# koesterlab/microphaser

Measured on AMD Instinct MI355X. Metric: peptide-windows/s (somatic, 9-mer), higher is better.
Workload: dtype u64

## Files before the change

### microphaser_amd/csrc/capi.cpp

```cpp
#include "../../include/microphaser_hip.h"

#include <cstdio>
#include <cstdlib>
#include <cstring>
#include <chrono>
#include <unistd.h>
#include <cerrno>
#include <fstream>
#include <iostream>
#include <memory>
#include <sstream>

#include "batch.hpp"
#include "consume.hpp"
#include "device.hpp"
#include "filter.hpp"
#include "pep.hpp"
#include "synth.hpp"

using namespace mp;

#include "capi_types.hpp"


// ... 193 lines not shown
                    batch->w_wins_known = true;
                }
                const uint64_t w_steps = batch->w_steps;
                const uint64_t seq_steps = b.steps.size() - w_steps, seq_wins = b.wins.size() - batch->w_wins;
                const double wfrac = b.wins.empty() ? 0.0 : double(batch->w_wins) / double(b.wins.size());
                const uint64_t groups_w = uint64_t(double(t.n_groups) * wfrac), groups_seq = t.n_groups - groups_w;
                const uint64_t read_bytes = 20 + 16ull * b.mask_words;
                st->k2seq_ms = t.k2seq_ms; st->k2a_ms = t.k2a_ms; st->k2w_ms = t.k2w_ms; st->k2win_ms = t.k2win_ms;
                st->n_steps_seq = seq_steps; st->n_steps_w = w_steps; st->n_adm = b.n_adm;
                const uint64_t rowrec = b.lane_on ? sizeof(RowRecA) + 8 : 0;
                if (!batch->adm_known) {
                    for (const ExonW& e : b.exons_w) { if (e.consumers & EW_WAVE) batch->adm_wave += e.n_reads; if (e.consumers & EW_LANE) batch->adm_lane += e.n_reads; }
                    batch->adm_known = true;
                }
                st->bytes_k2a = b.n_adm * read_bytes + batch->adm_wave * sizeof(AdmEntry) + batch->adm_lane * rowrec + b.exons_w.size() * sizeof(ExonW);
                uint64_t wave_steps = 0;
                for (const PodVec<WChunk>* list : {&b.wchunks, &b.wchunks_m, &b.wchunks_d}) for (const WChunk& c : *list) wave_steps += c.n_steps;
                const double wave_share = w_steps ? double(wave_steps) / double(w_steps) : 0.0;
                const uint64_t lane_wins = b.winw.size(), wave_wins = batch->w_wins - std::min<uint64_t>(batch->w_wins, lane_wins);
                const uint64_t groups_l = batch->w_wins ? uint64_t(double(groups_w) * double(lane_wins) / double(batch->w_wins)) : 0;
                st->k2l_ms = t.k2l_ms; st->n_windows_lane = lane_wins; st->n_windows_wave = wave_wins;
                const uint64_t listed_l = t.n_k3 > (t.n_groups - groups_l) ? t.n_k3 - (t.n_groups - groups_l) : 0;
                st->bytes_k2l = lane_wins * (sizeof(WinW) + 4 + sizeof(WinDyn)) + batch->adm_lane * rowrec + groups_l * sizeof(Group) + listed_l * 16;
                st->bytes_k2w = wave_steps * (sizeof(Step) + 7) + uint64_t(double(b.n_adm) * wave_share) * (read_bytes + sizeof(AdmEntry)) +
                                wave_wins * sizeof(WinDyn) + (groups_w - groups_l) * (sizeof(Group) + 16);
                st->bytes_k2seq = seq_steps * sizeof(Step) + (b.steps.empty() ? 0 : uint64_t(double(b.r_pos.size()) * double(seq_steps) / double(b.steps.size()))) * read_bytes +
                                  seq_wins * sizeof(WinDyn) + groups_seq * (sizeof(Group) + 16);
                st->bytes_k2 = st->bytes_k2a + st->bytes_k2l + st->bytes_k2w + st->bytes_k2seq;
            }
            st->n_groups_k3 = t.n_k3;
// ... 334 lines not shown
```

### microphaser_amd/csrc/device.cpp

```cpp
#include "device.hpp"
#include <chrono>
#include <cstdio>
#include <algorithm>

#include <algorithm>
#include <cstdlib>
#include <cstring>
#include <thread>

namespace mp {

[[noreturn]] void throw_hip(hipError_t e, const char* file, int line) {
    throw Error(std::string("HIP error: ") + hipGetErrorString(e) + " at " + file + ":" + std::to_string(line));
}
#define HIP_OK(x) do { hipError_t e_ = (x); if (e_ != hipSuccess) throw_hip(e_, __FILE__, __LINE__); } while (0)

DeviceContext::DeviceContext(int device) : device_(device) {
    int n = 0;
    hipError_t e = hipGetDeviceCount(&n);
    if (e != hipSuccess || n == 0) throw Error("no HIP device available: the phasing hot path needs an MI355X (gfx950); there is no CPU fallback");
    if (device < 0 || device >= n) throw Error("invalid HIP device index " + std::to_string(device));
    HIP_OK(hipSetDevice(device));
    HIP_OK(hipStreamCreateWithFlags(&stream_, hipStreamNonBlocking));
    for (auto& ev : ev_) HIP_OK(hipEventCreate(&ev));
// ... 271 lines not shown
    d_.tx_first_stop = static_cast<uint32_t*>(dalloc(size_t(d_.n_tx) * 4)); allocs_.push_back(d_.tx_first_stop);
    max_rows_bound_ = b.max_rows_bound;
    last_slots_ = last_recs_ = last_want_ = last_k3a_ = last_k3b_ = last_k3c_ = last_k3d_ = 0;
    rpl_ = 1;
    while (rpl_ < 16 && uint32_t(64 * rpl_) < max_rows_bound_) rpl_ *= 2;
    const uint64_t waves = b.wchunks.size() + b.segs.size() + b.wchunks_m.size() * (1 + b.rows_per_lane_w) + b.wchunks_d.size() * 16;
    uint64_t g_need = uint64_t(d_.n_wins) * 6 + waves * 256 + 4096;
    uint64_t r_need = g_need / 3 + waves * 128 + 4096;
    if (b.normal) { g_need += waves * 1024; r_need = g_need; }
    glog_ = 12; rlog_ = 12;
    while ((uint64_t(NPART) << glog_) < g_need + g_need / 4) glog_++;
    while ((uint64_t(NPART) << rlog_) < r_need + r_need / 4) rlog_++;
    if (std::getenv("MP_TEST_SMALL_CAPS")) glog_ = rlog_ = 8;
    d_.win_blobs = nullptr;
    if (!b.normal && d_.n_wins) { d_.win_blobs = static_cast<WinBlob*>(dalloc(size_t(d_.n_wins) * sizeof(WinBlob))); allocs_.push_back(d_.win_blobs); }
    d_.exons_a = nullptr; d_.adm_map = nullptr;
    if (b.n_adm) {
        d_.exons_a = static_cast<ExonA*>(dalloc(size_t(d_.n_exons_w) * sizeof(ExonA))); allocs_.push_back(d_.exons_a);
        d_.adm_map = static_cast<AdmMap*>(dalloc(size_t(b.n_adm) * sizeof(AdmMap))); allocs_.push_back(d_.adm_map);
    }
    const double ms_inputs = ms_since(t_up0);
    alloc_outputs();
    const double ms_alloc = ms_since(t_up0);
    uint64_t up_bytes = 0;
    for (const XferSeg& sgm : pending_up_) up_bytes += sgm.bytes;
    if (dbg) {
        std::vector<uint64_t> sz;
        for (const XferSeg& sgm : pending_up_) sz.push_back(sgm.bytes);
        std::sort(sz.rbegin(), sz.rend());
        std::fprintf(stderr, "[mp]   upload: %zu arrays, %.2f GB; the largest (MB):", pending_up_.size(), double(up_bytes) / 1e9);
        for (size_t k = 0; k < sz.size() && k < 14; k++) std::fprintf(stderr, " %.0f", double(sz[k]) / 1e6);
        std::fprintf(stderr, "\n[mp]   upload sizes (MB): reads fields %.0f, seq pool %.0f, cigar %.0f, ref %.0f, steps %.0f (+ side arrays %.0f), wins %.0f, win_cols %.0f, winw %.0f\n",
                     double(b.r_pos.size()) * (4 * 7 + 8 * 3) / 1e6, double(b.seq_pool.size()) / 1e6, double(b.cigar_pool.size()) * 4 / 1e6, double(b.ref_pool.size()) / 1e6,
                     double(b.steps.size()) * sizeof(Step) / 1e6, double(b.steps.size()) * 13 / 1e6 + double(b.step_aux.size()) * sizeof(b.step_aux[0]) / 1e6,
                     double(b.wins.size()) * sizeof(WinStatic) / 1e6, double(b.win_cols.size()) * sizeof(WinCol) / 1e6, double(b.winw.size()) * (sizeof(WinW) + 4) / 1e6);
    }
    xfer(pending_up_, true);
    pending_up_.clear();
    if (dbg) std::fprintf(stderr, "[mp]   upload: %u hipMalloc calls took %.1f ms in all; %u blocks came from the context's pool\n", alloc_calls_, alloc_ms_, alloc_reused_);
    if (dbg)
        std::fprintf(stderr, "[mp]   upload: release of the previous batch %.1f ms, per-read table + input allocations %.1f ms, result arenas %.1f ms, copies %.1f ms\n",
                     ms_free, ms_inputs - ms_free, ms_alloc - ms_inputs, ms_since(t_up0) - ms_alloc);
    launch_k0_read_variants(d_, stream_);
    launch_k0_pack_admission(d_, stream_);
    if (d_.win_blobs) launch_k0_pack_windows(d_, stream_);
    HIP_OK(hipStreamSynchronize(stream_));
    pool_trim(false);
}

void DeviceContext::alloc_outputs() {
    if ((uint64_t(NPART) << glog_) > 0x7FFFFFFFull || (uint64_t(NPART) << rlog_) > 0x7FFFFFFFull)
        throw Error("result buffers exceed 2^31 slots: split the batch by genes");
    free_outputs();
    group_cap_ = uint64_t(NPART) << glog_;
    rec_cap_ = uint64_t(NPART) << rlog_;
    auto oalloc = [&](size_t bytes) { void* p = dalloc(bytes); out_allocs_.push_back(p); out_bytes_ += bytes; return p; };
    d_.groups = static_cast<Group*>(oalloc(group_cap_ * sizeof(Group)));
    d_.k3_items = static_cast<uint4*>(oalloc(2 * group_cap_ * sizeof(uint4)));
    d_.gsum = static_cast<GroupSum*>(oalloc(group_cap_ * sizeof(GroupSum)));
    d_.recs = static_cast<uint8_t*>(oalloc(rec_cap_ * d_.rec_stride));
    d_.want_recs = static_cast<uint32_t*>(oalloc(rec_cap_ * 4));
    d_.group_part_log2 = glog_;
    d_.rec_part_log2 = rlog_;
    d_.group_cap = group_cap_;
    d_.rec_cap = rec_cap_;
}

void DeviceContext::run(RunTiming& t) {
    HIP_OK(hipSetDevice(device_));
    t = RunTiming();
    for (int attempt = 0; attempt < 8; attempt++) {
        t.attempts = uint32_t(attempt + 1);
        t.rows_per_lane = rpl_;
        HIP_OK(hipMemsetAsync(d_.cursors, 0, (NPART * 32 + 16) * 8, stream_));
        HIP_OK(hipMemsetAsync(d_.win_dyn, 0, size_t(d_.n_wins) * sizeof(WinDyn), side_[0]));
        HIP_OK(hipMemsetAsync(d_.tx_first_stop, 0xFF, size_t(d_.n_tx) * 4, side_[0]));
        HIP_OK(hipEventRecord(cleared_, side_[0]));
        HIP_OK(hipEventRecord(ev_[0], stream_));
        launch_k1_pileup_bits(d_, stream_);
        HIP_OK(hipEventRecord(ev_[1], stream_));
        HIP_OK(hipStreamWaitEvent(stream_, cleared_, 0));
        HIP_OK(hipEventRecord(fork_[0], stream_));
        HIP_OK(hipStreamWaitEvent(side_[2], fork_[0], 0));
        launch_k2_window_replay(d_, rpl_, side_[2]);
        HIP_OK(hipEventRecord(join_[2], side_[2]));
        HIP_OK(hipEventRecord(ev_[5], stream_));
        launch_k2_admission(d_, stream_);
        HIP_OK(hipEventRecord(ev_[6], stream_));
// ... 145 lines not shown
```

### microphaser_amd/csrc/device.hpp

```cpp
#pragma once
#include <string>
#include <vector>

#include "batch.hpp"
#include "kernels.hpp"

namespace mp {

struct HostResults {
    PodVec<WinDyn> win_dyn;
    PodVec<Group> groups;
    PodVec<GroupSum> gsum;
    PodVec<uint8_t> recs;
    uint32_t seq_cap = 48, rec_stride = 128;
    uint32_t group_part_log2 = 0, rec_part_log2 = 0;
    uint64_t group_prefix[NPART + 1] = {0}, rec_prefix[NPART + 1] = {0};
    size_t gidx(uint64_t slot) const { return size_t(group_prefix[slot >> group_part_log2] + (slot & ((1ull << group_part_log2) - 1))); }
    size_t ridx(uint64_t i) const { return size_t(rec_prefix[i >> rec_part_log2] + (i & ((1ull << rec_part_log2) - 1))); }
    const Group& grp(uint64_t slot) const { return groups[gidx(slot)]; }
    const GroupSum& gsm(uint64_t slot) const { return gsum[gidx(slot)]; }
    const HapRecHdr* rec(uint64_t i) const { return reinterpret_cast<const HapRecHdr*>(recs.data() + ridx(i) * rec_stride); }
    const uint8_t* rec_seq(uint64_t i) const { return recs.data() + ridx(i) * rec_stride + 32; }
    const uint8_t* rec_germ(uint64_t i) const { return recs.data() + ridx(i) * rec_stride + 32 + seq_cap; }
    uint64_t n_group_slots = 0, n_recs = 0;
};

struct RunTiming {
    float k1_ms = 0, k2_ms = 0, k3_ms = 0, k3b_ms = 0, total_ms = 0;
    float k2seq_ms = 0, k2a_ms = 0, k2l_ms = 0, k2w_ms = 0;
    float k2win_ms = 0;
    uint64_t n_group_slots = 0, n_recs = 0, n_groups = 0, n_k3 = 0, n_k3a = 0, n_k3c = 0, n_k3d = 0, n_rec_slots = 0;
    int rows_per_lane = 1;
    uint32_t attempts = 0;
};

class DeviceContext {
  public:
    explicit DeviceContext(int device);
    ~DeviceContext();
    DeviceContext(const DeviceContext&) = delete;
    DeviceContext& operator=(const DeviceContext&) = delete;

    void upload(const Batch& b);
    void run(RunTiming& t);
    void download(HostResults& r);
    void free_batch();
    int device() const { return device_; }
    uint64_t hbm_bytes() const { return hbm_bytes_; }
// ... 42 lines not shown
```

### microphaser_amd/csrc/kernels.hip

```cpp
#include <hip/hip_runtime.h>

#include <algorithm>
#include <cstdlib>
#include <type_traits>

#include "kernels.hpp"

namespace mp {

#ifndef MP_KPART
#define MP_KPART -1
#endif
#define MP_IN_PART(n) (MP_KPART == -1 || MP_KPART == (n))
#define HIP_CHECK_LAUNCH() \
    do { hipError_t e_ = hipGetLastError(); if (e_ != hipSuccess) { throw_hip(e_, __FILE__, __LINE__); } } while (0)

[[noreturn]] void throw_hip(hipError_t e, const char* file, int line);

#if MP_IN_PART(0)
__global__ __launch_bounds__(256) void k0_read_variants(DeviceBatch d) {
    const uint32_t i = blockIdx.x * 256u + threadIdx.x;
    if (i >= d.n_reads) return;
    uint32_t lo = 0, hi = d.n_genes;
    while (hi - lo > 1) {
// ... 62 lines not shown
    }
    return -1;
}

__device__ __forceinline__ uint8_t decode_base4(uint32_t code) {
    const uint64_t lo = 0x565352474d43413dull, hi = 0x4e42444b48595754ull;
    return uint8_t(((code & 8) ? hi : lo) >> (8 * (code & 7)));
}

constexpr uint32_t K1_LANES = 4;
static_assert(K1_LANES == 4, "the group's lanes combine their bits with quad permutes");
constexpr uint32_t K1_PAY_DW = 32;
constexpr uint32_t K1_PAY_STRIDE = 33;
struct __attribute__((packed, aligned(4))) K1Quad { uint32_t x, y, z, w; };

template <int W>
__global__ __launch_bounds__(256) void k1_pileup_bits(DeviceBatch d) {
    __shared__ uint32_t pay[(256 / K1_LANES) * K1_PAY_STRIDE];
    const uint64_t t = uint64_t(blockIdx.x) * 256u + threadIdx.x;
    const uint32_t sub = threadIdx.x & (K1_LANES - 1);
    const uint64_t i_raw = t / K1_LANES;
    const bool valid = i_raw < d.n_reads;
    const uint32_t i = valid ? uint32_t(i_raw) : d.n_reads - 1;
    const uint2 rv = d.r_var[i];
    const uint32_t vfirst = rv.x;
    const uint32_t rpos = d.r_pos[i], rend = d.r_end[i], lseq = d.r_lseq[i], ncig = d.r_ncig[i];
    const uint32_t* cig = d.cigar_pool + d.r_cigoff[i];
    const uint32_t* lowq = reinterpret_cast<const uint32_t*>(d.seq_pool + d.r_seqoff[i]);
    const uint32_t nlq = (lseq + 31) >> 5;
    const uint8_t* seq4 = reinterpret_cast<const uint8_t*>(lowq + nlq);
    const uint32_t cover_end = max(rend, rpos + lseq);
    const uint32_t maxn = min(rv.y, 64u * W);
    uint32_t* const slot = pay + (threadIdx.x / K1_LANES) * K1_PAY_STRIDE;
// ... 81 lines not shown
        ncov += __popc(acc_c);
#pragma unroll
        for (int w = 0; w < W; w++)
            if ((b0 >> 6) == uint32_t(w)) { sup[w] |= uint64_t(acc_s) << (b0 & 63u); lq[w] |= uint64_t(acc_q) << (b0 & 63u); }
        more = more && acc_c == 0xFFFFFFFFu;
    }
    };
    if (!any_long) run_batches(std::false_type{});
    else run_batches(std::true_type{});
    if (valid && sub == 0) {
        d.r_ncov[i] = ncov;
#pragma unroll
        for (int w = 0; w < W; w++) {
            d.r_sup[uint64_t(i) * W + w] = sup[w];
            d.r_lq[uint64_t(i) * W + w] = lq[w];
        }
    }
}

enum : uint32_t { ST_EMPTY = 0, ST_PENDING = 1, ST_ROW = 2, ST_MASK = 3, RF_BAD = 4, RF_SL = 8, RF_F1 = 16 };

__device__ __forceinline__ uint32_t rdlane(uint32_t v, uint32_t l) { return __builtin_amdgcn_readlane(v, l); }
__device__ __forceinline__ uint32_t lanes_below(uint64_t mask, uint32_t lane) { return __popcll(mask & ((1ull << lane) - 1ull)); }
__device__ __forceinline__ uint64_t wave_claim(unsigned long long* cur, unsigned long long want, uint64_t part_lo) {
    unsigned long long base = 0;
    if (threadIdx.x == 0) base = atomicAdd(cur, want);
    const uint32_t blo = rdlane(uint32_t(base), 0), bhi = rdlane(uint32_t(base >> 32), 0);
    return part_lo + ((uint64_t(bhi) << 32) | blo);
}

// ... 487 lines not shown
            w[8] = uint32_t(bits); w[9] = uint32_t(bits >> 32);
        }
    }
    return __ballot(lane < nb && ((w[5] >> 8) & SF_PRINT) && !k2l_takes(d.lane_on != 0, w[7] >> 16, w[7] & 0xFFFF));
}

#if MP_IN_PART(0)
__global__ __launch_bounds__(256) void k0_pack_admission(DeviceBatch d) {
    const uint64_t i = uint64_t(blockIdx.x) * 256u + threadIdx.x;
    if (i < d.n_exons_w) {
        const ExonW e = d.exons_w[i];
        ExonA a;
        a.step_off = e.step_off; a.n_steps = e.n_steps; a.unit_steps = e.unit_steps; a.sso0 = e.sso0;
        a.sso1 = e.sso1; a.first_key_lo = e.first_key_lo; a.range = e.range; a.tr0 = e.tr0;
        a.f0 = e.f0; a.sl_f_lo = e.sl_f_lo; a.sl_f_hi = e.sl_f_hi; a.flags = (e.strand ? 1u : 0u) | (e.consumers << 8);
        a.adm_off = e.adm_off; a.read0 = e.rbase + e.read_lo; a.wlen_min = e.wlen_min; a.pad1 = 0;
        d.exons_a[i] = a;
    }
    if (i < d.n_adm) {
        uint32_t lo = 0, hi = d.n_exons_w;
        while (hi - lo > 1) {
            const uint32_t mid = lo + (hi - lo) / 2;
            if (d.exons_w[mid].adm_off <= i) lo = mid; else hi = mid;
        }
        const ExonW* e = d.exons_w + lo;
        AdmMap m;
        m.exon = lo;
        m.read = e->rbase + e->read_lo + uint32_t(i - e->adm_off);
        d.adm_map[i] = m;
    }
}
void launch_k0_pack_admission(const DeviceBatch& d, hipStream_t stream) {
    if (!d.n_adm) return;
    const uint64_t n = d.n_adm > d.n_exons_w ? d.n_adm : d.n_exons_w;
    hipLaunchKernelGGL(k0_pack_admission, dim3(uint32_t((n + 255) / 256)), dim3(256), 0, stream, d);
    HIP_CHECK_LAUNCH();
}
#endif

template <int W>
__global__ __launch_bounds__(64) void k2a_admission_flat(DeviceBatch d) {
    struct In {
        bool on, rev, go;
        uint32_t entry, t;
        AdmMap xr;
        ExonA e;
        uint32_t start, end, rvl;
        uint64_t sup[W], dirty[W];
        uint32_t s_sso, s_col_hi, s_w4, s_w5, nc;
        AdmEntry out;
    };
    const uint32_t n_adm = uint32_t(d.n_adm);
    auto load_entry = [&](In& I, uint32_t tile) __attribute__((always_inline)) {
        const uint64_t entry = uint64_t(tile) * 64u + threadIdx.x;
        I.on = entry < n_adm;
        I.entry = I.on ? uint32_t(entry) : n_adm - 1u;
        I.xr = d.adm_map[I.entry];
    };
    auto load_fields = [&](In& I) __attribute__((always_inline)) {
        const uint4* ep = reinterpret_cast<const uint4*>(d.exons_a + I.xr.exon);
        const uint4 q0 = ep[0], q1 = ep[1], q2 = ep[2], q3 = ep[3];
        const uint32_t gi = I.xr.read;
        I.start = d.r_pos[gi]; I.end = d.r_end[gi]; I.rvl = d.r_varlo[gi];
#pragma unroll
        for (int w = 0; w < W; w++) { I.sup[w] = d.r_sup[uint64_t(gi) * W + w]; I.dirty[w] = d.r_lq[uint64_t(gi) * W + w]; }
        I.e.step_off = q0.x; I.e.n_steps = q0.y; I.e.unit_steps = q0.z; I.e.sso0 = q0.w;
        I.e.sso1 = q1.x; I.e.first_key_lo = q1.y; I.e.range = q1.z; I.e.tr0 = q1.w;
        I.e.f0 = q2.x; I.e.sl_f_lo = q2.y; I.e.sl_f_hi = q2.z; I.e.flags = q2.w;
        I.e.adm_off = q3.x; I.e.read0 = q3.y; I.e.wlen_min = q3.z;
    };
    auto load_step = [&](In& I, uint32_t si) __attribute__((always_inline)) {
        const uint32_t* sp = reinterpret_cast<const uint32_t*>(d.steps + si);
        I.s_sso = sp[0]; I.s_col_hi = sp[2]; I.s_w4 = sp[4]; I.s_w5 = sp[5];
        I.nc = d.step_ncols[si];
    };
    auto eval_step = [&](In& I, uint32_t si) __attribute__((always_inline)) -> bool {
        const uint32_t s_wlen = (I.s_w4 >> 16) & 0xFFu, s_nadd = I.s_w5 & 0xFFu;
        const uint32_t tlo = I.s_col_hi - I.nc, thi = I.s_col_hi - s_nadd;
        uint32_t flo = tlo, fhi = thi;
        if (I.rev) { flo = I.e.f0 - (thi - 1 - I.e.tr0); fhi = I.e.f0 - (tlo - I.e.tr0) + 1; }
        if (thi <= tlo) flo = fhi = 0;
        const bool encloses = !(I.end < I.s_sso + s_wlen) & !(I.start > I.s_sso);
        const bool clean = !mask_hits<W>(I.dirty, flo, fhi, I.rvl);
        const bool ok = encloses & clean;
        I.out.ord = ok ? si : I.out.ord;
        I.out.seen_lo = ok ? tlo : I.out.seen_lo;
        return ok;
    };
    auto first_step = [&](In& I) __attribute__((always_inline)) {
        const ExonA& e = I.e;
        I.rev = (e.flags & 1u) != 0;
#pragma unroll
        for (int w = 0; w < W; w++) I.dirty[w] |= I.sup[w] & bit_range(e.sl_f_lo, e.sl_f_hi, I.rvl + 64u * w);
        I.out.ord = 0xFFFFFFFFu; I.out.seen_lo = 0;
        I.go = false; I.t = 0;
        const uint32_t start = I.start;
        if (!I.rev) {
            if (start >= e.first_key_lo && start <= e.sso0) {
                I.go = true;
            } else if (start > e.sso0 && e.n_steps > 1 && start >= e.sso1) {
                uint32_t t = 1 + (start - e.sso1);
                if (t < e.unit_steps) { I.go = true; I.t = t; }
                else if (t < e.n_steps) {
                    uint32_t s_t = d.steps[e.step_off + t].sso;
                    while (s_t > start && t > 1) s_t = d.steps[e.step_off + --t].sso;
                    while (s_t < start && t + 1 < e.n_steps) s_t = d.steps[e.step_off + ++t].sso;
                    if (s_t == start) { I.go = true; I.t = t; }
                }
            }
        } else {
            const uint32_t top = start + e.range;
            uint32_t t = e.sso0 > top ? e.sso0 - top : 0;
            if (t >= e.unit_steps) {
                if (t >= e.n_steps) t = e.n_steps - 1;
                while (t > 0 && d.steps[e.step_off + t - 1].sso <= top) t--;
                while (t < e.n_steps && d.steps[e.step_off + t].sso > top) t++;
            }
            if (t < e.unit_steps) {
                const uint32_t need = e.sso0 + e.wlen_min > I.end ? e.sso0 + e.wlen_min - I.end : 0u;
                t = max(t, min(need, e.unit_steps));
            }
            I.go = t < e.n_steps; I.t = I.go ? t : 0;
        }
    };
    auto finish = [&](In& I) __attribute__((always_inline)) {
        const ExonA& e = I.e;
        if (I.go) {
            if (!I.rev) eval_step(I, e.step_off + I.t);
            else {
                uint32_t t = I.t;
                for (;;) {
                    if (I.s_sso < I.start) break;
                    if (eval_step(I, e.step_off + t)) break;
                    if (++t >= e.n_steps) break;
                    load_step(I, e.step_off + t);
                }
            }
        }
        if (!I.on) return;
        const uint32_t consumers = e.flags >> 8;
        if (consumers & EW_WAVE) d.adm[I.entry] = I.out;
        if constexpr (W == 1) {
            if (d.lane_on && (consumers & EW_LANE)) {
                uint32_t bad_from = 0xFFFFFFFFu;
                if (I.out.ord != 0xFFFFFFFFu) {
                    const uint64_t dm = I.dirty[0];
                    if (!I.rev) {
                        const uint32_t from = max(I.out.seen_lo, I.rvl), sh = from - I.rvl;
                        const uint64_t m = sh < 64 ? dm >> sh : 0ull;
                        if (m) bad_from = from + uint32_t(__builtin_ctzll(m));
                    } else {
                        const uint32_t f_hi = e.f0 - (I.out.seen_lo - e.tr0);
                        if (f_hi >= I.rvl) {
                            const uint32_t rel = f_hi - I.rvl;
                            const uint64_t m = rel >= 63 ? dm : (dm & ((2ull << rel) - 1ull));
                            if (m) bad_from = e.tr0 + (e.f0 - (I.rvl + 63u - uint32_t(__builtin_clzll(m))));
                        }
                    }
                }
                RowRecA a;
                a.key = I.rev ? ~I.start : I.end;
                a.ord = I.out.ord;
                a.bad_from = bad_from;
                a.rvl = I.rvl;
                d.rr_a[I.entry] = a;
                d.rr_sup[I.entry] = I.sup[0];
            }
        }
    };
    In in0;
    load_entry(in0, blockIdx.x);
    load_fields(in0);
    first_step(in0);
    load_step(in0, in0.e.step_off + in0.t);
    finish(in0);
}

template <int HB, int STAGE_>
__global__ __launch_bounds__(64) void k2l_window_lanes(DeviceBatch d, uint32_t first, uint32_t count) {
    constexpr bool HASH = HB > 8;
    constexpr uint32_t NW = HASH ? 64u : (1u << HB) / 4;
    constexpr uint32_t EMPTY = 0xFFFFFFFFu;
    constexpr uint32_t STAGE = STAGE_ ? STAGE_ : 1;
    static_assert(STAGE_ == 0 || STAGE_ > int(K2L_MAX_ROWS), "a window's candidate reads must fit one stage pass, or the staging loop never ends");
    __shared__ uint32_t hist[NW * 64];
    __shared__ uint4 st_a[STAGE];
    __shared__ uint64_t st_s[STAGE];
    const uint32_t lane = threadIdx.x;
#pragma unroll 4
    for (uint32_t t = 0; t < NW; t++) hist[t * 64 + lane] = HASH ? EMPTY : 0u;
// ... 1779 lines not shown
#pragma unroll
    for (int k = 0; k < 6; k++) idw[k] = reinterpret_cast<const uint32_t*>(idp - id_mis)[k];
    const uint64_t id60 = haplotype_id60<SEQ_CAP>(d, active, sq, seq_len, T.id_off, T.id_len, idw, id_mis, win_sso,
                                                  lds_blk + threadIdx.x * (K3B_BUF_WORDS + 1), byte_text);
    if (active) {
        rec[2] = uint32_t(id60);
        rec[3] = uint32_t(id60 >> 32);
    }
    }
}

#if MP_IN_PART(0)
void launch_k1_pileup_bits(const DeviceBatch& d, hipStream_t stream) {
    if (d.n_reads == 0) return;
    dim3 grid(uint32_t((uint64_t(d.n_reads) * K1_LANES + 255) / 256)), block(256);
    switch (d.mask_words) {
        case 1: hipLaunchKernelGGL(k1_pileup_bits<1>, grid, block, 0, stream, d); break;
        case 2: hipLaunchKernelGGL(k1_pileup_bits<2>, grid, block, 0, stream, d); break;
        case 3: case 4: {
            DeviceBatch d4 = d;
            if (d.mask_words == 3) throw_hip(hipErrorInvalidValue, __FILE__, __LINE__);
            hipLaunchKernelGGL(k1_pileup_bits<4>, grid, block, 0, stream, d4);
            break;
        }
        default: throw_hip(hipErrorInvalidValue, __FILE__, __LINE__);
    }
    HIP_CHECK_LAUNCH();
}

#endif
#if MP_IN_PART(1)
void launch_k2_window_replay(const DeviceBatch& d, int rows_per_lane, hipStream_t stream) {
    if (d.n_segs == 0) return;
    dim3 grid(d.n_segs), block(64);
    if (d.normal) {
#define K2N_CASE(R) case R: if (d.normal_large) hipLaunchKernelGGL((k2n_window_replay<R, 512, 2048>), grid, block, 0, stream, d); \
                            else hipLaunchKernelGGL((k2n_window_replay<R, 128, 512>), grid, block, 0, stream, d); break;
// ... 7 lines not shown
    }
    switch (rows_per_lane) {
        case 1: hipLaunchKernelGGL(k2_window_replay<1>, grid, block, 0, stream, d); break;
        case 2: hipLaunchKernelGGL(k2_window_replay<2>, grid, block, 0, stream, d); break;
        case 4: hipLaunchKernelGGL(k2_window_replay<4>, grid, block, 0, stream, d); break;
        case 8: hipLaunchKernelGGL(k2_window_replay<8>, grid, block, 0, stream, d); break;
        case 16: hipLaunchKernelGGL(k2_window_replay<16>, grid, block, 0, stream, d); break;
        default: throw_hip(hipErrorInvalidValue, __FILE__, __LINE__);
    }
    HIP_CHECK_LAUNCH();
}

#endif
#if MP_IN_PART(0)
void launch_k2_admission(const DeviceBatch& d, hipStream_t stream) {
    if (!d.n_adm) return;
    const dim3 grid(uint32_t((d.n_adm + 63) / 64)), block(64);
    if (d.mask_words == 1) hipLaunchKernelGGL(k2a_admission_flat<1>, grid, block, 0, stream, d);
    else if (d.mask_words == 2) hipLaunchKernelGGL(k2a_admission_flat<2>, grid, block, 0, stream, d);
    else throw_hip(hipErrorInvalidValue, __FILE__, __LINE__);
    HIP_CHECK_LAUNCH();
}
#endif
#if MP_IN_PART(2)
template <int W>
static void launch_k2w_multi(const DeviceBatch& d, hipStream_t stream) {
    dim3 grid(d.n_wchunks_m), block(64);
    switch (d.rows_per_lane_w) {
        case 1: hipLaunchKernelGGL((k2w_window_rows_multi<1, W>), grid, block, 0, stream, d); break;
        case 2: hipLaunchKernelGGL((k2w_window_rows_multi<2, W>), grid, block, 0, stream, d); break;
        case 4: hipLaunchKernelGGL((k2w_window_rows_multi<4, W>), grid, block, 0, stream, d); break;
// ... 116 lines not shown
```

### microphaser_amd/csrc/kernels.hpp

```cpp
#pragma once
#include <hip/hip_runtime.h>

#include "plan.hpp"

namespace mp {

constexpr uint32_t NPART = 64;

struct DeviceBatch {
    const uint32_t *g_read_off, *g_var_off, *g_start;
    const uint64_t* g_ref_off;
    uint32_t n_genes, n_genes_pad_;
    uint2* r_var;
    const uint32_t *r_pos, *r_end, *r_lseq, *r_ncig, *r_dup;
    const uint64_t *r_cigoff, *r_seqoff;
    const uint32_t* cigar_pool;
    const uint8_t* seq_pool;
    const uint32_t *v_pos, *v_info, *v_len, *v_insoff, *v_rev2fwd;
    const uint8_t* ins_pool;
    const uint8_t* ref_pool;
    const TxDev* tx;
    const Step* steps;
    const uint16_t* step_aux;
    const WinStatic* wins;
    const WinCol* win_cols;
    ExonA* exons_a;
    AdmMap* adm_map;
    WinBlob* win_blobs;
    const uint8_t* str_pool;
    const SegDev* segs;
    const uint32_t* seg_order;
    uint32_t n_segs;
    const ExonW* exons_w;
    const WChunk* wchunks;
    const WChunk* wchunks_m;
    const WChunk* wchunks_d;
    const uint8_t* step_ncols;
    const uint32_t* step_rlo;
    const uint16_t* step_rn;
    const uint64_t* v_sombits;
    AdmEntry* adm;
    RowRecA* rr_a;
    uint64_t* rr_sup;
    const WinW* winw;
    const uint32_t* lane_win;
    const uint32_t* win_trivial;
    const uint32_t* win_walk;
    const uint32_t* win_simple;
    uint32_t n_lane_small, n_lane_all, lane_on, n_lane_mid;
    uint32_t n_exons_w, n_wchunks, n_wchunks_m, n_wchunks_d;
    uint32_t rows_per_lane_w;
    uint64_t n_adm;
    uint32_t n_reads, n_tx, n_wins, mask_words;
    uint32_t normal;
    uint32_t normal_large;
    uint32_t timing_skip_ids;
    uint32_t timing_pad_;
    const uint32_t* r_varlo;
    uint32_t* r_ncov;
    uint64_t *r_sup, *r_lq;
    WinDyn* win_dyn;
    Group* groups;
    uint4* k3_items;
    uint32_t* want_recs;
    unsigned long long* cursors;
    uint32_t group_part_log2, rec_part_log2;
    uint64_t group_cap, rec_cap;
    uint32_t* err;
    GroupSum* gsum;
    uint8_t* recs;
    uint32_t seq_cap, rec_stride;
    uint32_t* tx_first_stop;
};

void launch_k0_pack_admission(const DeviceBatch& d, hipStream_t stream);
void launch_k0_read_variants(const DeviceBatch& d, hipStream_t stream);
void launch_k0_pack_windows(const DeviceBatch& d, hipStream_t stream);
void launch_k1_pileup_bits(const DeviceBatch& d, hipStream_t stream);
void launch_k2_window_replay(const DeviceBatch& d, int rows_per_lane, hipStream_t stream);
void launch_k2_admission(const DeviceBatch& d, hipStream_t stream);
void launch_k2_window_rows(const DeviceBatch& d, hipStream_t stream);
void launch_k2_window_lanes(const DeviceBatch& d, hipStream_t stream_small, hipStream_t stream_wide, hipStream_t stream_hash);
void launch_k3_window_seq(const DeviceBatch& d, uint64_t max_list_a, uint64_t max_list_b, uint64_t max_list_c, uint64_t max_list_d,
                          hipStream_t stream_a, hipStream_t stream_b, hipStream_t stream_c, hipStream_t stream_d);
void launch_k3b_haplotype_ids(const DeviceBatch& d, uint64_t max_recs, hipStream_t stream);

}
```

### microphaser_amd/csrc/plan.hpp

```cpp
#pragma once
#include <cstdint>

namespace mp {

enum : uint32_t {
    VI_KIND_MASK = 0x3,
    VI_GERMLINE = 1u << 2,
    VI_FS_SHIFT = 3,
    VI_FS_MASK = 0x3u << 3,
    VI_ALT_SHIFT = 8,
};

struct TxDev {
    uint32_t gene;
    uint32_t step_off;
    uint32_t n_steps;
    uint32_t strand;
    uint32_t sl_lo, sl_hi;
    uint32_t id_off, id_len;
};

struct SegDev {
    uint32_t tx;
    uint32_t step_off;
// ... 12 lines not shown
    uint32_t tr0, f0;
    uint32_t sl_f_lo, sl_f_hi;
    uint32_t strand;
    uint32_t rbase, vbase;
    uint32_t sso0, sso1;
    uint32_t unit_steps;
    uint32_t consumers;
    uint32_t wlen_min;
};
enum : uint32_t { EW_WAVE = 1,
                  EW_LANE = 2 };
struct ExonA {
    uint32_t step_off, n_steps, unit_steps, sso0;
    uint32_t sso1, first_key_lo, range, tr0;
    uint32_t f0, sl_f_lo, sl_f_hi, flags;
    uint32_t adm_off, read0, wlen_min, pad1;
};
static_assert(sizeof(ExonA) == 64, "ExonA layout");
struct AdmMap { uint32_t exon, read; };

struct WChunk {
    uint32_t exon, step_first, n_steps, pad;
};
struct AdmEntry {
    uint32_t ord;
    uint32_t seen_lo;
};

constexpr uint32_t K2L_MAX_COLS = 8;
constexpr uint32_t K2L_SMALL_COLS = 6;
constexpr uint32_t K2L_MAX_ROWS = 255;
constexpr uint32_t K2L_HASH_COLS = 16;
constexpr uint32_t K2L_HASH_ROWS = 63;
#if defined(__HIPCC__) || defined(__CUDACC__)
// ... 142 lines not shown
```

Before: 2.481 billion.

## Fuse read admission into the pileup kernel using per-block sorted admission items

Admission evaluation, previously a separate k2a kernel that re-read each read's position, end, varlo and support/dirty masks from global memory, now runs at the tail of k1_pileup_bits. There it takes those values from shared memory staged by the same workgroup. A one-time setup step radix-sorts the admission map by read block with rocprim and builds per-block offsets, so each K1 workgroup knows which admission items belong to its 64 reads. This removes a kernel launch and global re-reads of per-read masks. In exchange it adds setup cost (sort, temporary hipMalloc, sync), extra device buffers, and serial admission work on only one wave per K1 block.

```diff
diff --git a/microphaser_amd/csrc/capi.cpp b/microphaser_amd/csrc/capi.cpp
--- a/microphaser_amd/csrc/capi.cpp
+++ b/microphaser_amd/csrc/capi.cpp
@@ -231,6 +231,10 @@
                     batch->adm_known = true;
                 }
                 st->bytes_k2a = b.n_adm * read_bytes + batch->adm_wave * sizeof(AdmEntry) + batch->adm_lane * rowrec + b.exons_w.size() * sizeof(ExonW);
+                if (t.fused_adm) {
+                    st->bytes_k1 += st->bytes_k2a - b.n_adm * read_bytes;
+                    st->bytes_k2a = 0;
+                }
                 uint64_t wave_steps = 0;
                 for (const PodVec<WChunk>* list : {&b.wchunks, &b.wchunks_m, &b.wchunks_d}) for (const WChunk& c : *list) wave_steps += c.n_steps;
                 const double wave_share = w_steps ? double(wave_steps) / double(w_steps) : 0.0;
diff --git a/microphaser_amd/csrc/device.cpp b/microphaser_amd/csrc/device.cpp
--- a/microphaser_amd/csrc/device.cpp
+++ b/microphaser_amd/csrc/device.cpp
@@ -309,10 +309,15 @@
     if (std::getenv("MP_TEST_SMALL_CAPS")) glog_ = rlog_ = 8;
     d_.win_blobs = nullptr;
     if (!b.normal && d_.n_wins) { d_.win_blobs = static_cast<WinBlob*>(dalloc(size_t(d_.n_wins) * sizeof(WinBlob))); allocs_.push_back(d_.win_blobs); }
-    d_.exons_a = nullptr; d_.adm_map = nullptr;
+    d_.exons_a = nullptr; d_.adm_map = nullptr; d_.blk_items = nullptr; d_.blk_off = nullptr;
+    d_.fuse_adm = (b.n_adm && !b.normal && b.mask_words <= 2 && !std::getenv("MP_SPLIT_ADMISSION")) ? 1u : 0u;
     if (b.n_adm) {
         d_.exons_a = static_cast<ExonA*>(dalloc(size_t(d_.n_exons_w) * sizeof(ExonA))); allocs_.push_back(d_.exons_a);
         d_.adm_map = static_cast<AdmMap*>(dalloc(size_t(b.n_adm) * sizeof(AdmMap))); allocs_.push_back(d_.adm_map);
+        if (d_.fuse_adm) {
+            d_.blk_items = static_cast<AdmMap*>(dalloc(size_t(b.n_adm) * sizeof(AdmMap))); allocs_.push_back(d_.blk_items);
+            d_.blk_off = static_cast<uint32_t*>(dalloc((size_t(d_.n_reads) / K1_BLOCK_READS + 2) * 4)); allocs_.push_back(d_.blk_off);
+        }
     }
     const double ms_inputs = ms_since(t_up0);
     alloc_outputs();
@@ -338,6 +343,7 @@
                      ms_free, ms_inputs - ms_free, ms_alloc - ms_inputs, ms_since(t_up0) - ms_alloc);
     launch_k0_read_variants(d_, stream_);
     launch_k0_pack_admission(d_, stream_);
+    if (d_.fuse_adm) launch_k0_block_admission(d_, stream_);
     if (d_.win_blobs) launch_k0_pack_windows(d_, stream_);
     HIP_OK(hipStreamSynchronize(stream_));
     pool_trim(false);
@@ -367,6 +373,7 @@
     for (int attempt = 0; attempt < 8; attempt++) {
         t.attempts = uint32_t(attempt + 1);
         t.rows_per_lane = rpl_;
+        t.fused_adm = d_.fuse_adm != 0;
         HIP_OK(hipMemsetAsync(d_.cursors, 0, (NPART * 32 + 16) * 8, stream_));
         HIP_OK(hipMemsetAsync(d_.win_dyn, 0, size_t(d_.n_wins) * sizeof(WinDyn), side_[0]));
         HIP_OK(hipMemsetAsync(d_.tx_first_stop, 0xFF, size_t(d_.n_tx) * 4, side_[0]));
diff --git a/microphaser_amd/csrc/device.hpp b/microphaser_amd/csrc/device.hpp
--- a/microphaser_amd/csrc/device.hpp
+++ b/microphaser_amd/csrc/device.hpp
@@ -32,6 +32,7 @@
     uint64_t n_group_slots = 0, n_recs = 0, n_groups = 0, n_k3 = 0, n_k3a = 0, n_k3c = 0, n_k3d = 0, n_rec_slots = 0;
     int rows_per_lane = 1;
     uint32_t attempts = 0;
+    bool fused_adm = false;
 };
 
 class DeviceContext {
diff --git a/microphaser_amd/csrc/kernels.hip b/microphaser_amd/csrc/kernels.hip
--- a/microphaser_amd/csrc/kernels.hip
+++ b/microphaser_amd/csrc/kernels.hip
@@ -5,6 +5,10 @@
 #include <type_traits>
 
 #include "kernels.hpp"
+
+#if !defined(MP_KPART) || MP_KPART == 0
+#include <rocprim/device/device_radix_sort.hpp>
+#endif
 
 namespace mp {
 
@@ -100,9 +104,19 @@
 constexpr uint32_t K1_PAY_STRIDE = 33;
 struct __attribute__((packed, aligned(4))) K1Quad { uint32_t x, y, z, w; };
 
-template <int W>
+template <int W> struct AdmIn;
+template <int W> __device__ __forceinline__ void adm_load_exon(const DeviceBatch& d, AdmIn<W>& I);
+template <int W> __device__ __forceinline__ void adm_load_step(const DeviceBatch& d, AdmIn<W>& I, uint32_t si);
+template <int W> __device__ __forceinline__ void adm_first_step(const DeviceBatch& d, AdmIn<W>& I);
+template <int W> __device__ __forceinline__ void adm_finish(const DeviceBatch& d, AdmIn<W>& I);
+static_assert(256 / K1_LANES == K1_BLOCK_READS, "a K1 workgroup handles K1_BLOCK_READS consecutive reads");
+
+template <int W, bool FUSE>
 __global__ __launch_bounds__(256) void k1_pileup_bits(DeviceBatch d) {
     __shared__ uint32_t pay[(256 / K1_LANES) * K1_PAY_STRIDE];
+    constexpr int TW = FUSE ? W : 1, TN = FUSE ? int(K1_BLOCK_READS) : 1;
+    __shared__ uint64_t t_sup[TN * TW], t_lq[TN * TW];
+    __shared__ uint32_t t_start[TN], t_end[TN], t_vfirst[TN];
     const uint64_t t = uint64_t(blockIdx.x) * 256u + threadIdx.x;
     const uint32_t sub = threadIdx.x & (K1_LANES - 1);
     const uint64_t i_raw = t / K1_LANES;
@@ -214,6 +228,32 @@
         for (int w = 0; w < W; w++) {
             d.r_sup[uint64_t(i) * W + w] = sup[w];
             d.r_lq[uint64_t(i) * W + w] = lq[w];
+        }
+    }
+    if constexpr (FUSE) {
+        if (sub == 0) {
+            const uint32_t r = threadIdx.x / K1_LANES;
+            t_start[r] = rpos; t_end[r] = rend; t_vfirst[r] = vfirst;
+#pragma unroll
+            for (int w = 0; w < W; w++) { t_sup[r * W + w] = sup[w]; t_lq[r * W + w] = lq[w]; }
+        }
+        __syncthreads();
+        if (threadIdx.x >= 64) return;
+        const uint32_t it0 = d.blk_off[blockIdx.x], it1 = d.blk_off[blockIdx.x + 1];
+        for (uint32_t base = it0; base < it1; base += 64) {
+            AdmIn<W> I;
+            const uint32_t at = base + threadIdx.x;
+            I.on = at < it1;
+            I.xr = d.blk_items[I.on ? at : it1 - 1u];
+            adm_load_exon<W>(d, I);
+            const uint32_t r = I.xr.read & (K1_BLOCK_READS - 1u);
+            I.entry = I.e.adm_off + (I.xr.read - I.e.read0);
+            I.start = t_start[r]; I.end = t_end[r]; I.rvl = t_vfirst[r] - I.e.vbase;
+#pragma unroll
+            for (int w = 0; w < W; w++) { I.sup[w] = t_sup[r * W + w]; I.dirty[w] = t_lq[r * W + w]; }
+            adm_first_step<W>(d, I);
+            adm_load_step<W>(d, I, I.e.step_off + I.t);
+            adm_finish<W>(d, I);
         }
     }
 }
@@ -731,7 +771,7 @@
         a.step_off = e.step_off; a.n_steps = e.n_steps; a.unit_steps = e.unit_steps; a.sso0 = e.sso0;
         a.sso1 = e.sso1; a.first_key_lo = e.first_key_lo; a.range = e.range; a.tr0 = e.tr0;
         a.f0 = e.f0; a.sl_f_lo = e.sl_f_lo; a.sl_f_hi = e.sl_f_hi; a.flags = (e.strand ? 1u : 0u) | (e.consumers << 8);
-        a.adm_off = e.adm_off; a.read0 = e.rbase + e.read_lo; a.wlen_min = e.wlen_min; a.pad1 = 0;
+        a.adm_off = e.adm_off; a.read0 = e.rbase + e.read_lo; a.wlen_min = e.wlen_min; a.vbase = e.vbase;
         d.exons_a[i] = a;
     }
     if (i < d.n_adm) {
@@ -747,6 +787,48 @@
         d.adm_map[i] = m;
     }
 }
+__global__ __launch_bounds__(256) void k0_block_keys(const AdmMap* adm_map, uint64_t n_adm, uint32_t* keys) {
+    const uint64_t i = uint64_t(blockIdx.x) * 256u + threadIdx.x;
+    if (i < n_adm) keys[i] = adm_map[i].read / K1_BLOCK_READS;
+}
+__global__ __launch_bounds__(256) void k0_block_offsets(const uint32_t* keys, uint64_t n_adm, uint32_t n_blocks, uint32_t* blk_off) {
+    const uint32_t b = blockIdx.x * 256u + threadIdx.x;
+    if (b > n_blocks) return;
+    uint64_t lo = 0, hi = n_adm;
+    while (lo < hi) {
+        const uint64_t mid = lo + (hi - lo) / 2;
+        if (keys[mid] < b) lo = mid + 1; else hi = mid;
+    }
+    blk_off[b] = uint32_t(lo);
+}
+void launch_k0_block_admission(const DeviceBatch& d, hipStream_t stream) {
+    if (!d.n_adm || !d.blk_items || !d.blk_off) return;
+    const size_t n = size_t(d.n_adm);
+    const uint32_t n_blocks = (d.n_reads + K1_BLOCK_READS - 1) / K1_BLOCK_READS;
+    uint32_t key_bits = 1;
+    while (key_bits < 32 && (uint64_t(1) << key_bits) < n_blocks) key_bits++;
+    const uint64_t* vals_in = reinterpret_cast<const uint64_t*>(d.adm_map);
+    uint64_t* vals_out = reinterpret_cast<uint64_t*>(d.blk_items);
+    size_t ws_bytes = 0;
+    hipError_t e = rocprim::radix_sort_pairs(nullptr, ws_bytes, static_cast<uint32_t*>(nullptr), static_cast<uint32_t*>(nullptr), vals_in, vals_out, n, 0u, key_bits, stream);
+    if (e != hipSuccess) throw_hip(e, __FILE__, __LINE__);
+    const size_t key_bytes = (n * 4 + 255) & ~size_t(255);
+    char* tmp = nullptr;
+    e = hipMalloc(&tmp, 2 * key_bytes + ws_bytes + 256);
+    if (e != hipSuccess) throw_hip(e, __FILE__, __LINE__);
+    uint32_t* keys = reinterpret_cast<uint32_t*>(tmp);
+    uint32_t* keys_sorted = reinterpret_cast<uint32_t*>(tmp + key_bytes);
+    hipLaunchKernelGGL(k0_block_keys, dim3(uint32_t((n + 255) / 256)), dim3(256), 0, stream, d.adm_map, uint64_t(n), keys);
+    e = hipGetLastError();
+    if (e == hipSuccess) e = rocprim::radix_sort_pairs(tmp + 2 * key_bytes, ws_bytes, keys, keys_sorted, vals_in, vals_out, n, 0u, key_bits, stream);
+    if (e == hipSuccess) {
+        hipLaunchKernelGGL(k0_block_offsets, dim3(n_blocks / 256 + 1), dim3(256), 0, stream, keys_sorted, uint64_t(n), n_blocks, d.blk_off);
+        e = hipGetLastError();
+    }
+    if (e == hipSuccess) e = hipStreamSynchronize(stream);
+    (void)hipFree(tmp);
+    if (e != hipSuccess) throw_hip(e, __FILE__, __LINE__);
+}
 void launch_k0_pack_admission(const DeviceBatch& d, hipStream_t stream) {
     if (!d.n_adm) return;
     const uint64_t n = d.n_adm > d.n_exons_w ? d.n_adm : d.n_exons_w;
@@ -756,141 +838,145 @@
 #endif
 
 template <int W>
+struct AdmIn {
+    bool on, rev, go;
+    uint32_t entry, t;
+    AdmMap xr;
+    ExonA e;
+    uint32_t start, end, rvl;
+    uint64_t sup[W], dirty[W];
+    uint32_t s_sso, s_col_hi, s_w4, s_w5, nc;
+    AdmEntry out;
+};
+template <int W>
+__device__ __forceinline__ void adm_load_exon(const DeviceBatch& d, AdmIn<W>& I) {
+    const uint4* ep = reinterpret_cast<const uint4*>(d.exons_a + I.xr.exon);
+    const uint4 q0 = ep[0], q1 = ep[1], q2 = ep[2], q3 = ep[3];
+    I.e.step_off = q0.x; I.e.n_steps = q0.y; I.e.unit_steps = q0.z; I.e.sso0 = q0.w;
+    I.e.sso1 = q1.x; I.e.first_key_lo = q1.y; I.e.range = q1.z; I.e.tr0 = q1.w;
+    I.e.f0 = q2.x; I.e.sl_f_lo = q2.y; I.e.sl_f_hi = q2.z; I.e.flags = q2.w;
+    I.e.adm_off = q3.x; I.e.read0 = q3.y; I.e.wlen_min = q3.z; I.e.vbase = q3.w;
+}
+template <int W>
+__device__ __forceinline__ void adm_load_step(const DeviceBatch& d, AdmIn<W>& I, uint32_t si) {
+    const uint32_t* sp = reinterpret_cast<const uint32_t*>(d.steps + si);
+    I.s_sso = sp[0]; I.s_col_hi = sp[2]; I.s_w4 = sp[4]; I.s_w5 = sp[5];
+    I.nc = d.step_ncols[si];
+}
+template <int W>
+__device__ __forceinline__ bool adm_eval_step(AdmIn<W>& I, uint32_t si) {
+    const uint32_t s_wlen = (I.s_w4 >> 16) & 0xFFu, s_nadd = I.s_w5 & 0xFFu;
+    const uint32_t tlo = I.s_col_hi - I.nc, thi = I.s_col_hi - s_nadd;
+    uint32_t flo = tlo, fhi = thi;
+    if (I.rev) { flo = I.e.f0 - (thi - 1 - I.e.tr0); fhi = I.e.f0 - (tlo - I.e.tr0) + 1; }
+    if (thi <= tlo) flo = fhi = 0;
+    const bool encloses = !(I.end < I.s_sso + s_wlen) & !(I.start > I.s_sso);
+    const bool clean = !mask_hits<W>(I.dirty, flo, fhi, I.rvl);
+    const bool ok = encloses & clean;
+    I.out.ord = ok ? si : I.out.ord;
+    I.out.seen_lo = ok ? tlo : I.out.seen_lo;
+    return ok;
+}
+template <int W>
+__device__ __forceinline__ void adm_first_step(const DeviceBatch& d, AdmIn<W>& I) {
+    const ExonA& e = I.e;
+    I.rev = (e.flags & 1u) != 0;
+#pragma unroll
+    for (int w = 0; w < W; w++) I.dirty[w] |= I.sup[w] & bit_range(e.sl_f_lo, e.sl_f_hi, I.rvl + 64u * w);
+    I.out.ord = 0xFFFFFFFFu; I.out.seen_lo = 0;
+    I.go = false; I.t = 0;
+    const uint32_t start = I.start;
+    if (!I.rev) {
+        if (start >= e.first_key_lo && start <= e.sso0) {
+            I.go = true;
+        } else if (start > e.sso0 && e.n_steps > 1 && start >= e.sso1) {
+            uint32_t t = 1 + (start - e.sso1);
+            if (t < e.unit_steps) { I.go = true; I.t = t; }
+            else if (t < e.n_steps) {
+                uint32_t s_t = d.steps[e.step_off + t].sso;
+                while (s_t > start && t > 1) s_t = d.steps[e.step_off + --t].sso;
+                while (s_t < start && t + 1 < e.n_steps) s_t = d.steps[e.step_off + ++t].sso;
+                if (s_t == start) { I.go = true; I.t = t; }
+            }
+        }
+    } else {
+        const uint32_t top = start + e.range;
+        uint32_t t = e.sso0 > top ? e.sso0 - top : 0;
+        if (t >= e.unit_steps) {
+            if (t >= e.n_steps) t = e.n_steps - 1;
+            while (t > 0 && d.steps[e.step_off + t - 1].sso <= top) t--;
+            while (t < e.n_steps && d.steps[e.step_off + t].sso > top) t++;
+        }
+        if (t < e.unit_steps) {
+            const uint32_t need = e.sso0 + e.wlen_min > I.end ? e.sso0 + e.wlen_min - I.end : 0u;
+            t = max(t, min(need, e.unit_steps));
+        }
+        I.go = t < e.n_steps; I.t = I.go ? t : 0;
+    }
+}
+template <int W>
+__device__ __forceinline__ void adm_finish(const DeviceBatch& d, AdmIn<W>& I) {
+    const ExonA& e = I.e;
+    if (I.go) {
+        if (!I.rev) adm_eval_step<W>(I, e.step_off + I.t);
+        else {
+            uint32_t t = I.t;
+            for (;;) {
+                if (I.s_sso < I.start) break;
+                if (adm_eval_step<W>(I, e.step_off + t)) break;
+                if (++t >= e.n_steps) break;
+                adm_load_step<W>(d, I, e.step_off + t);
+            }
+        }
+    }
+    if (!I.on) return;
+    const uint32_t consumers = e.flags >> 8;
+    if (consumers & EW_WAVE) d.adm[I.entry] = I.out;
+    if constexpr (W == 1) {
+        if (d.lane_on && (consumers & EW_LANE)) {
+            uint32_t bad_from = 0xFFFFFFFFu;
+            if (I.out.ord != 0xFFFFFFFFu) {
+                const uint64_t dm = I.dirty[0];
+                if (!I.rev) {
+                    const uint32_t from = max(I.out.seen_lo, I.rvl), sh = from - I.rvl;
+                    const uint64_t m = sh < 64 ? dm >> sh : 0ull;
+                    if (m) bad_from = from + uint32_t(__builtin_ctzll(m));
+                } else {
+                    const uint32_t f_hi = e.f0 - (I.out.seen_lo - e.tr0);
+                    if (f_hi >= I.rvl) {
+                        const uint32_t rel = f_hi - I.rvl;
+                        const uint64_t m = rel >= 63 ? dm : (dm & ((2ull << rel) - 1ull));
+                        if (m) bad_from = e.tr0 + (e.f0 - (I.rvl + 63u - uint32_t(__builtin_clzll(m))));
+                    }
+                }
+            }
+            RowRecA a;
+            a.key = I.rev ? ~I.start : I.end;
+            a.ord = I.out.ord;
+            a.bad_from = bad_from;
+            a.rvl = I.rvl;
+            d.rr_a[I.entry] = a;
+            d.rr_sup[I.entry] = I.sup[0];
+        }
+    }
+}
+
+template <int W>
 __global__ __launch_bounds__(64) void k2a_admission_flat(DeviceBatch d) {
-    struct In {
-        bool on, rev, go;
-        uint32_t entry, t;
-        AdmMap xr;
-        ExonA e;
-        uint32_t start, end, rvl;
-        uint64_t sup[W], dirty[W];
-        uint32_t s_sso, s_col_hi, s_w4, s_w5, nc;
-        AdmEntry out;
-    };
     const uint32_t n_adm = uint32_t(d.n_adm);
-    auto load_entry = [&](In& I, uint32_t tile) __attribute__((always_inline)) {
-        const uint64_t entry = uint64_t(tile) * 64u + threadIdx.x;
-        I.on = entry < n_adm;
-        I.entry = I.on ? uint32_t(entry) : n_adm - 1u;
-        I.xr = d.adm_map[I.entry];
-    };
-    auto load_fields = [&](In& I) __attribute__((always_inline)) {
-        const uint4* ep = reinterpret_cast<const uint4*>(d.exons_a + I.xr.exon);
-        const uint4 q0 = ep[0], q1 = ep[1], q2 = ep[2], q3 = ep[3];
-        const uint32_t gi = I.xr.read;
-        I.start = d.r_pos[gi]; I.end = d.r_end[gi]; I.rvl = d.r_varlo[gi];
-#pragma unroll
-        for (int w = 0; w < W; w++) { I.sup[w] = d.r_sup[uint64_t(gi) * W + w]; I.dirty[w] = d.r_lq[uint64_t(gi) * W + w]; }
-        I.e.step_off = q0.x; I.e.n_steps = q0.y; I.e.unit_steps = q0.z; I.e.sso0 = q0.w;
-        I.e.sso1 = q1.x; I.e.first_key_lo = q1.y; I.e.range = q1.z; I.e.tr0 = q1.w;
-        I.e.f0 = q2.x; I.e.sl_f_lo = q2.y; I.e.sl_f_hi = q2.z; I.e.flags = q2.w;
-        I.e.adm_off = q3.x; I.e.read0 = q3.y; I.e.wlen_min = q3.z;
-    };
-    auto load_step = [&](In& I, uint32_t si) __attribute__((always_inline)) {
-        const uint32_t* sp = reinterpret_cast<const uint32_t*>(d.steps + si);
-        I.s_sso = sp[0]; I.s_col_hi = sp[2]; I.s_w4 = sp[4]; I.s_w5 = sp[5];
-        I.nc = d.step_ncols[si];
-    };
-    auto eval_step = [&](In& I, uint32_t si) __attribute__((always_inline)) -> bool {
-        const uint32_t s_wlen = (I.s_w4 >> 16) & 0xFFu, s_nadd = I.s_w5 & 0xFFu;
-        const uint32_t tlo = I.s_col_hi - I.nc, thi = I.s_col_hi - s_nadd;
-        uint32_t flo = tlo, fhi = thi;
-        if (I.rev) { flo = I.e.f0 - (thi - 1 - I.e.tr0); fhi = I.e.f0 - (tlo - I.e.tr0) + 1; }
-        if (thi <= tlo) flo = fhi = 0;
-        const bool encloses = !(I.end < I.s_sso + s_wlen) & !(I.start > I.s_sso);
-        const bool clean = !mask_hits<W>(I.dirty, flo, fhi, I.rvl);
-        const bool ok = encloses & clean;
-        I.out.ord = ok ? si : I.out.ord;
-        I.out.seen_lo = ok ? tlo : I.out.seen_lo;
-        return ok;
-    };
-    auto first_step = [&](In& I) __attribute__((always_inline)) {
-        const ExonA& e = I.e;
-        I.rev = (e.flags & 1u) != 0;
-#pragma unroll
-        for (int w = 0; w < W; w++) I.dirty[w] |= I.sup[w] & bit_range(e.sl_f_lo, e.sl_f_hi, I.rvl + 64u * w);
-        I.out.ord = 0xFFFFFFFFu; I.out.seen_lo = 0;
-        I.go = false; I.t = 0;
-        const uint32_t start = I.start;
-        if (!I.rev) {
-            if (start >= e.first_key_lo && start <= e.sso0) {
-                I.go = true;
-            } else if (start > e.sso0 && e.n_steps > 1 && start >= e.sso1) {
-                uint32_t t = 1 + (start - e.sso1);
-                if (t < e.unit_steps) { I.go = true; I.t = t; }
-                else if (t < e.n_steps) {
-                    uint32_t s_t = d.steps[e.step_off + t].sso;
-                    while (s_t > start && t > 1) s_t = d.steps[e.step_off + --t].sso;
-                    while (s_t < start && t + 1 < e.n_steps) s_t = d.steps[e.step_off + ++t].sso;
-                    if (s_t == start) { I.go = true; I.t = t; }
-                }
-            }
-        } else {
-            const uint32_t top = start + e.range;
-            uint32_t t = e.sso0 > top ? e.sso0 - top : 0;
-            if (t >= e.unit_steps) {
-                if (t >= e.n_steps) t = e.n_steps - 1;
-                while (t > 0 && d.steps[e.step_off + t - 1].sso <= top) t--;
-                while (t < e.n_steps && d.steps[e.step_off + t].sso > top) t++;
-            }
-            if (t < e.unit_steps) {
-                const uint32_t need = e.sso0 + e.wlen_min > I.end ? e.sso0 + e.wlen_min - I.end : 0u;
-                t = max(t, min(need, e.unit_steps));
-            }
-            I.go = t < e.n_steps; I.t = I.go ? t : 0;
-        }
-    };
-    auto finish = [&](In& I) __attribute__((always_inline)) {
-        const ExonA& e = I.e;
-        if (I.go) {
-            if (!I.rev) eval_step(I, e.step_off + I.t);
-            else {
-                uint32_t t = I.t;
-                for (;;) {
-                    if (I.s_sso < I.start) break;
-                    if (eval_step(I, e.step_off + t)) break;
-                    if (++t >= e.n_steps) break;
-                    load_step(I, e.step_off + t);
-                }
-            }
-        }
-        if (!I.on) return;
-        const uint32_t consumers = e.flags >> 8;
-        if (consumers & EW_WAVE) d.adm[I.entry] = I.out;
-        if constexpr (W == 1) {
-            if (d.lane_on && (consumers & EW_LANE)) {
-                uint32_t bad_from = 0xFFFFFFFFu;
-                if (I.out.ord != 0xFFFFFFFFu) {
-                    const uint64_t dm = I.dirty[0];
-                    if (!I.rev) {
-                        const uint32_t from = max(I.out.seen_lo, I.rvl), sh = from - I.rvl;
-                        const uint64_t m = sh < 64 ? dm >> sh : 0ull;
-                        if (m) bad_from = from + uint32_t(__builtin_ctzll(m));
-                    } else {
-                        const uint32_t f_hi = e.f0 - (I.out.seen_lo - e.tr0);
-                        if (f_hi >= I.rvl) {
-                            const uint32_t rel = f_hi - I.rvl;
-                            const uint64_t m = rel >= 63 ? dm : (dm & ((2ull << rel) - 1ull));
-                            if (m) bad_from = e.tr0 + (e.f0 - (I.rvl + 63u - uint32_t(__builtin_clzll(m))));
-                        }
-                    }
-                }
-                RowRecA a;
-                a.key = I.rev ? ~I.start : I.end;
-                a.ord = I.out.ord;
-                a.bad_from = bad_from;
-                a.rvl = I.rvl;
-                d.rr_a[I.entry] = a;
-                d.rr_sup[I.entry] = I.sup[0];
-            }
-        }
-    };
-    In in0;
-    load_entry(in0, blockIdx.x);
-    load_fields(in0);
-    first_step(in0);
-    load_step(in0, in0.e.step_off + in0.t);
-    finish(in0);
+    AdmIn<W> in0;
+    const uint64_t entry = uint64_t(blockIdx.x) * 64u + threadIdx.x;
+    in0.on = entry < n_adm;
+    in0.entry = in0.on ? uint32_t(entry) : n_adm - 1u;
+    in0.xr = d.adm_map[in0.entry];
+    adm_load_exon<W>(d, in0);
+    const uint32_t gi = in0.xr.read;
+    in0.start = d.r_pos[gi]; in0.end = d.r_end[gi]; in0.rvl = d.r_varlo[gi];
+#pragma unroll
+    for (int w = 0; w < W; w++) { in0.sup[w] = d.r_sup[uint64_t(gi) * W + w]; in0.dirty[w] = d.r_lq[uint64_t(gi) * W + w]; }
+    adm_first_step<W>(d, in0);
+    adm_load_step<W>(d, in0, in0.e.step_off + in0.t);
+    adm_finish<W>(d, in0);
 }
 
 template <int HB, int STAGE_>
@@ -2700,13 +2786,18 @@
 void launch_k1_pileup_bits(const DeviceBatch& d, hipStream_t stream) {
     if (d.n_reads == 0) return;
     dim3 grid(uint32_t((uint64_t(d.n_reads) * K1_LANES + 255) / 256)), block(256);
+    if (d.fuse_adm && (d.mask_words > 2 || !d.blk_items || !d.blk_off)) throw_hip(hipErrorInvalidValue, __FILE__, __LINE__);
     switch (d.mask_words) {
-        case 1: hipLaunchKernelGGL(k1_pileup_bits<1>, grid, block, 0, stream, d); break;
-        case 2: hipLaunchKernelGGL(k1_pileup_bits<2>, grid, block, 0, stream, d); break;
+        case 1: if (d.fuse_adm) hipLaunchKernelGGL((k1_pileup_bits<1, true>), grid, block, 0, stream, d);
+                else hipLaunchKernelGGL((k1_pileup_bits<1, false>), grid, block, 0, stream, d);
+                break;
+        case 2: if (d.fuse_adm) hipLaunchKernelGGL((k1_pileup_bits<2, true>), grid, block, 0, stream, d);
+                else hipLaunchKernelGGL((k1_pileup_bits<2, false>), grid, block, 0, stream, d);
+                break;
         case 3: case 4: {
             DeviceBatch d4 = d;
             if (d.mask_words == 3) throw_hip(hipErrorInvalidValue, __FILE__, __LINE__);
-            hipLaunchKernelGGL(k1_pileup_bits<4>, grid, block, 0, stream, d4);
+            hipLaunchKernelGGL((k1_pileup_bits<4, false>), grid, block, 0, stream, d4);
             break;
         }
         default: throw_hip(hipErrorInvalidValue, __FILE__, __LINE__);
@@ -2744,7 +2835,7 @@
 #endif
 #if MP_IN_PART(0)
 void launch_k2_admission(const DeviceBatch& d, hipStream_t stream) {
-    if (!d.n_adm) return;
+    if (!d.n_adm || d.fuse_adm) return;
     const dim3 grid(uint32_t((d.n_adm + 63) / 64)), block(64);
     if (d.mask_words == 1) hipLaunchKernelGGL(k2a_admission_flat<1>, grid, block, 0, stream, d);
     else if (d.mask_words == 2) hipLaunchKernelGGL(k2a_admission_flat<2>, grid, block, 0, stream, d);
diff --git a/microphaser_amd/csrc/kernels.hpp b/microphaser_amd/csrc/kernels.hpp
--- a/microphaser_amd/csrc/kernels.hpp
+++ b/microphaser_amd/csrc/kernels.hpp
@@ -26,6 +26,8 @@
     const WinCol* win_cols;
     ExonA* exons_a;
     AdmMap* adm_map;
+    AdmMap* blk_items;
+    uint32_t* blk_off;
     WinBlob* win_blobs;
     const uint8_t* str_pool;
     const SegDev* segs;
@@ -55,7 +57,7 @@
     uint32_t normal;
     uint32_t normal_large;
     uint32_t timing_skip_ids;
-    uint32_t timing_pad_;
+    uint32_t fuse_adm;
     const uint32_t* r_varlo;
     uint32_t* r_ncov;
     uint64_t *r_sup, *r_lq;
@@ -74,6 +76,7 @@
 };
 
 void launch_k0_pack_admission(const DeviceBatch& d, hipStream_t stream);
+void launch_k0_block_admission(const DeviceBatch& d, hipStream_t stream);
 void launch_k0_read_variants(const DeviceBatch& d, hipStream_t stream);
 void launch_k0_pack_windows(const DeviceBatch& d, hipStream_t stream);
 void launch_k1_pileup_bits(const DeviceBatch& d, hipStream_t stream);
diff --git a/microphaser_amd/csrc/plan.hpp b/microphaser_amd/csrc/plan.hpp
--- a/microphaser_amd/csrc/plan.hpp
+++ b/microphaser_amd/csrc/plan.hpp
@@ -50,10 +50,11 @@
     uint32_t step_off, n_steps, unit_steps, sso0;
     uint32_t sso1, first_key_lo, range, tr0;
     uint32_t f0, sl_f_lo, sl_f_hi, flags;
-    uint32_t adm_off, read0, wlen_min, pad1;
+    uint32_t adm_off, read0, wlen_min, vbase;
 };
 static_assert(sizeof(ExonA) == 64, "ExonA layout");
 struct AdmMap { uint32_t exon, read; };
+constexpr uint32_t K1_BLOCK_READS = 64;
 
 struct WChunk {
     uint32_t exon, step_first, n_steps, pad;
```

After: 2.059 billion. 17.0% lower.
